# jaideepmurkute/Inference-Efficient-Vision-Models

Hardware: NVIDIA B200
Metric: pruned-INT8 ResNet-18 images/s @bs256 per GPU (synthetic 3x224x224) (higher is better)
Workload: dtype u8

## Files before the change

inference-efficient-vision-models_b200/csrc/conv_dual.cuh:

```cuda
#pragma once
#include "conv_tc.cuh"

namespace ievm {

struct ConvDualParams {
  void* out;
  const float* ep0;
  const float* ep1;
  int out_zp, out_lo;
  int fast_round;
  int relu;
  int32_t* dump_acc;
  float epc0[kEpConst];
  float epc1[kEpConst];
};

template <int kDtype, int kCluster>
__global__ void __launch_bounds__(kConvThreads, 1)
conv_dual_kernel(const __grid_constant__ CUtensorMap tmap_a, const __grid_constant__ CUtensorMap tmap_b,
                 const __grid_constant__ CUtensorMap tmap_b2, const __grid_constant__ ConvTcParams p,
                 const __grid_constant__ ConvDualParams x) {
  extern __shared__ uint8_t smem_raw[];
  const uint32_t raw_addr = smem_u32(smem_raw);
  uint8_t* smem = smem_raw + ((1024u - (raw_addr & 1023u)) & 1023u);

  const int kw = p.kw != 0 ? p.kw : p.ksize;
  const int stride_w = p.kw != 0 ? p.stride_w : p.stride;
  const int pad_w = p.kw != 0 ? p.pad_w : p.pad;
  const int num_kb = p.ksize * kw * p.kchunks;
  const int a_bytes = p.a_stage_bytes;
  const int b_bytes = (p.bn / kCluster) * p.kc_bytes;
  const int G = p.kb_group;
  const int slots = p.stages * G;
  const int b_slots = p.resident_b ? num_kb + p.kchunks : slots;
  uint8_t* sA = smem;
  uint8_t* sB = smem + slots * a_bytes;
  float* s_ep = reinterpret_cast<float*>(sB + b_slots * b_bytes);
  uint64_t* full_bar = reinterpret_cast<uint64_t*>(s_ep + 4 * p.cout_pad);
  uint64_t* empty_bar = full_bar + p.stages;
  uint64_t* tfull_bar = empty_bar + p.stages;
  uint64_t* tempty_bar = tfull_bar + kMaxAcc;
  uint64_t* bres_bar = tempty_bar + kMaxAcc;
  uint32_t* tmem_slot = reinterpret_cast<uint32_t*>(bres_bar + 1);

// ... 36 lines not shown
  tc_fence_before();
  __syncthreads();
  if (kCluster > 1) cluster_sync_all();
  tc_fence_after();
  const uint32_t tmem_base = *reinterpret_cast<volatile uint32_t*>(tmem_slot);
  griddep_launch_dependents();

  const int class_tiles = kCluster > 1 ? ((p.m_tiles + kCluster - 1) / kCluster) * p.n_tiles : p.m_tiles * p.n_tiles;
  const int total_tiles = 2 * class_tiles;
  const int tile_first = kCluster > 1 ? static_cast<int>(blockIdx.x) / kCluster : static_cast<int>(blockIdx.x);
  const int tile_step = kCluster > 1 ? static_cast<int>(gridDim.x) / kCluster : static_cast<int>(gridDim.x);
  const int hw = p.ho * p.wo;
  const int ctr_y = p.ksize >> 1, ctr_x = kw >> 1;

  if (warp == 0) {
    if (p.resident_b && elect_one()) {
      mbar_expect_tx(bres_bar, static_cast<uint32_t>((num_kb + p.kchunks) * b_bytes));
      for (int kb = 0; kb < num_kb; ++kb) tma_load_2d(sB + kb * b_bytes, &tmap_b, bres_bar, kb * p.kc_elems, 0);
      for (int ch = 0; ch < p.kchunks; ++ch)
        tma_load_2d(sB + (num_kb + ch) * b_bytes, &tmap_b2, bres_bar, ch * p.kc_elems, 0);
    }
    __syncwarp();
    griddep_wait_conv();
    const uint32_t tx_bytes = static_cast<uint32_t>(p.resident_b ? p.a_tx_bytes : p.a_tx_bytes + b_bytes);
    int stage = 0;
    uint32_t phase = 0;
    for (int tile = tile_first; tile < total_tiles; tile += tile_step) {
      const bool cls1 = tile >= class_tiles;
      const int ct = cls1 ? tile - class_tiles : tile;
      const int m_group = ct / p.n_tiles;
      const int n_tile = ct - m_group * p.n_tiles;
      const int m_tile = kCluster > 1 ? m_group * kCluster + static_cast<int>(crank) : m_group;
      const int m0 = m_tile * kTileM;
      const int img = fast_div(m0, hw, p.hw_magic);
      const int rem = m0 - img * hw;
      const int oy = fast_div(rem, p.wo, p.wo_magic);
      const int ox = rem - oy * p.wo;
      const int base_w = ox * stride_w - pad_w;
      const int base_h = oy * p.stride - p.pad;
      const int ty_lo = cls1 ? ctr_y : 0, ty_hi = cls1 ? ctr_y + 1 : p.ksize;
      const int tx_lo = cls1 ? ctr_x : 0, tx_hi = cls1 ? ctr_x + 1 : kw;
      const int nkb = cls1 ? p.kchunks : num_kb;
      const CUtensorMap* wmap = cls1 ? &tmap_b2 : &tmap_b;
      int kb = 0, g = 0;
      for (int ty = ty_lo; ty < ty_hi; ++ty) {
        for (int tx = tx_lo; tx < tx_hi; ++tx) {
// ... 41 lines not shown
    const uint32_t b_step = static_cast<uint32_t>(b_bytes) >> 4;
    const uint32_t idesc = p.idesc;
    auto mma = [&](uint32_t d, uint32_t a_lo, uint32_t b_lo, uint32_t accum) {
      if (kCluster > 1) {
        if (kDtype == kDtypeI8) umma_i8_lohi_pair(d, a_lo, b_lo, hi, idesc, accum);
        else umma_f16_lohi_pair(d, a_lo, b_lo, hi, idesc, accum);
      } else {
        if (kDtype == kDtypeI8) umma_i8_lohi(d, a_lo, b_lo, hi, idesc, accum);
        else umma_f16_lohi(d, a_lo, b_lo, hi, idesc, accum);
      }
    };
    if (p.resident_b) wait_or_die(bres_bar, 0, 0x500u, p.stuck_flag);
    for (int tile = tile_first; leader && tile < total_tiles; tile += tile_step) {
      const bool cls1 = tile >= class_tiles;
      const int nkb = cls1 ? p.kchunks : num_kb;
      const int b_first = cls1 ? num_kb : 0;
      wait_or_die(&tempty_bar[acc], acc_phase ^ 1u, 0x200u | acc, p.stuck_flag);
      tc_fence_after();
      const uint32_t d_tmem = tmem_base + static_cast<uint32_t>(acc * p.acc_stride);
      for (int kb0 = 0; kb0 < nkb; kb0 += G) {
        const int cnt = min(G, nkb - kb0);
        wait_or_die(&full_bar[stage], phase, 0x300u | stage, p.stuck_flag);
        tc_fence_after();
        if (elect_one()) {
          for (int g = 0; g < cnt; ++g) {
            const int kb = kb0 + g;
            const uint32_t a_lo = a_lo0 + static_cast<uint32_t>(stage * G + g) * a_step;
            const uint32_t b_lo = b_lo0 + static_cast<uint32_t>(p.resident_b ? b_first + kb : stage * G + g) * b_step;
            mma(d_tmem, a_lo, b_lo, kb != 0 ? 1u : 0u);
            mma(d_tmem, a_lo + 2, b_lo + 2, 1u);
            if (wide) {
              mma(d_tmem, a_lo + 4, b_lo + 4, 1u);
              mma(d_tmem, a_lo + 6, b_lo + 6, 1u);
            }
          }
          const bool last = kb0 + cnt == nkb;
          if (kCluster > 1) {
            umma_commit_pair(&empty_bar[stage]);
            if (last) umma_commit_pair(&tfull_bar[acc]);
          } else {
            umma_commit(&empty_bar[stage]);
            if (last) umma_commit(&tfull_bar[acc]);
          }
        }
        __syncwarp();
        if (++stage == p.stages) {
          stage = 0;
          phase ^= 1u;
        }
      }
      if (++acc == p.nacc) {
        acc = 0;
        acc_phase ^= 1u;
      }
    }
  } else {
    const int quad = warp & 3;
    const int groups = p.nacc < kGroupsMax ? p.nacc : kGroupsMax;
    const int group = ((warp - 2) >> 2) & (groups - 1);
    const int sub = ((warp - 2) >> 2) / groups;
    const int csub = kGroupsMax / groups;
    const int row = quad * 32 + lane;
    const int nchunks = p.bn >> 4;
    griddep_wait_conv();
    int acc_next = 0, seq = 0;
    uint32_t acc_phase_next = 0;
    for (int tile = tile_first; tile < total_tiles; tile += tile_step, ++seq) {
      const int acc = acc_next;
      const uint32_t acc_phase = acc_phase_next;
      if (++acc_next == p.nacc) {
        acc_next = 0;
        acc_phase_next ^= 1u;
      }
      if ((seq & (groups - 1)) != group) continue;
      const bool cls1 = tile >= class_tiles;
      const int ct = cls1 ? tile - class_tiles : tile;
      const int m_group = ct / p.n_tiles;
      const int n_tile = ct - m_group * p.n_tiles;
      const int m_tile = kCluster > 1 ? m_group * kCluster + static_cast<int>(crank) : m_group;
      const int m = m_tile * kTileM + row;
      const bool valid = m < p.m_total;
      const int n0 = n_tile * p.bn;
      uint8_t* out_row = static_cast<uint8_t*>(cls1 ? x.out : p.out) +
                         static_cast<size_t>(m) * p.out_pitch * (kDtype == kDtypeI8 ? 1 : 2);
      const float* e0 = s_ep + (cls1 ? 2 * p.cout_pad : 0);
      const float* e1 = e0 + p.cout_pad;
      const int zp = cls1 ? x.out_zp : p.out_zp;
      const int lo = cls1 ? x.out_lo : p.out_lo;
      const bool fast = (cls1 ? x.fast_round : p.fast_round) != 0;
      const bool relu = (cls1 ? x.relu : p.relu) != 0;
      int32_t* dump = cls1 ? x.dump_acc : p.dump_acc;

      wait_or_die(&tfull_bar[acc], acc_phase, 0x400u | acc, p.stuck_flag);
      tc_fence_after();
      const uint32_t t_row = tmem_base + (static_cast<uint32_t>(quad * 32) << 16) + static_cast<uint32_t>(acc * p.acc_stride);
      uint32_t va[16], vb[16];
      auto chunk = [&](const uint32_t (&v)[16], int c) {
        const int ch = n0 + c * 16;
        if (valid && dump != nullptr) {
          int4* d = reinterpret_cast<int4*>(dump + static_cast<size_t>(m) * p.dump_pitch + ch);
#pragma unroll
          for (int j = 0; j < 4; ++j)
            d[j] = make_int4(static_cast<int>(v[4 * j]), static_cast<int>(v[4 * j + 1]), static_cast<int>(v[4 * j + 2]),
                             static_cast<int>(v[4 * j + 3]));
        }
        if (kDtype == kDtypeI8) {
          const uint4 o = fast ? epilogue16_i8<true>(v, e0 + ch, e1 + ch, zp, lo) : epilogue16_i8<false>(v, e0 + ch, e1 + ch, zp, lo);
          if (valid) *reinterpret_cast<uint4*>(out_row + ch) = o;
        } else {
          __half* op = reinterpret_cast<__half*>(out_row) + ch;
          if (relu) epilogue16_f16<false, true>(v, e0 + ch, op, op, valid);
          else epilogue16_f16<false, false>(v, e0 + ch, op, op, valid);
        }
      };
      int c = sub;
      if (c < nchunks) tmem_ld_32x32b_x16(t_row + static_cast<uint32_t>(c * 16), va);
      while (c < nchunks) {
        tmem_ld_wait();
        if (c + csub < nchunks) tmem_ld_32x32b_x16(t_row + static_cast<uint32_t>((c + csub) * 16), vb);
        chunk(va, c);
        c += csub;
        if (c >= nchunks) break;
        tmem_ld_wait();
        if (c + csub < nchunks) tmem_ld_32x32b_x16(t_row + static_cast<uint32_t>((c + csub) * 16), va);
        chunk(vb, c);
        c += csub;
      }
      tc_fence_before();
      __syncwarp();
      if (lane == 0) {
        if (kCluster > 1 && !leader) mbar_arrive_remote(&tempty_bar[acc], 0u);
        else mbar_arrive(&tempty_bar[acc]);
      }
    }
  }

  tc_fence_before();
  __syncthreads();
  if (kCluster > 1) cluster_sync_all();
  if (warp == 1) {
    tc_fence_after();
    if (kCluster > 1) tmem_dealloc_pair(tmem_base, static_cast<uint32_t>(p.tmem_cols));
    else tmem_dealloc(tmem_base, static_cast<uint32_t>(p.tmem_cols));
  }
}

}
```

inference-efficient-vision-models_b200/csrc/conv_s2.cuh:

```cuda
#pragma once
#include "conv_dual.cuh"

namespace ievm {

__global__ void __launch_bounds__(kConvThreads, 1)
conv_s2_kernel(const __grid_constant__ CUtensorMap tmap_a, const __grid_constant__ CUtensorMap tmap_b,
               const __grid_constant__ CUtensorMap tmap_b2, const __grid_constant__ ConvTcParams p,
               const __grid_constant__ ConvDualParams x) {
  extern __shared__ uint8_t smem_raw[];
  const uint32_t raw_addr = smem_u32(smem_raw);
  uint8_t* smem = smem_raw + ((1024u - (raw_addr & 1023u)) & 1023u);

  constexpr int kRowBytes = 64;
  constexpr int kBlocks = 10;
  const int pb = p.phase_bytes;
  const int b_bytes = p.bn * kRowBytes;
  uint8_t* sA = smem;
  uint8_t* sB = smem + p.stages * p.a_stage_bytes + 1024;
  uint64_t* full_bar = reinterpret_cast<uint64_t*>(sB + kBlocks * b_bytes);
  uint64_t* empty_bar = full_bar + p.stages;
  uint64_t* tfull_bar = empty_bar + p.stages;
  uint64_t* tempty_bar = tfull_bar + kMaxAcc;
  uint64_t* bres_bar = tempty_bar + kMaxAcc;
  uint32_t* tmem_slot = reinterpret_cast<uint32_t*>(bres_bar + 1);

  const int warp = threadIdx.x >> 5;
  const int lane = threadIdx.x & 31;

  if (warp == 0 && lane == 0) {
    tma_prefetch_desc(&tmap_a);
    tma_prefetch_desc(&tmap_b);
// ... 15 lines not shown
  }
  tc_fence_before();
  __syncthreads();
  tc_fence_after();
  const uint32_t tmem_base = *reinterpret_cast<volatile uint32_t*>(tmem_slot);
  griddep_launch_dependents();

  int t_begin, t_end;
  {
    const int q = p.total_subs / static_cast<int>(gridDim.x), r = p.total_subs - q * static_cast<int>(gridDim.x);
    const int b = static_cast<int>(blockIdx.x);
    t_begin = b * q + (b < r ? b : r);
    t_end = t_begin + q + (b < r ? 1 : 0);
  }

  if (warp == 0) {
    if (elect_one()) {
      mbar_expect_tx(bres_bar, static_cast<uint32_t>(kBlocks * b_bytes));
      for (int kb = 0; kb < 9; ++kb) tma_load_2d(sB + kb * b_bytes, &tmap_b, bres_bar, kb * kRowBytes, 0);
      tma_load_2d(sB + 9 * b_bytes, &tmap_b2, bres_bar, 0, 0);
    }
    __syncwarp();
    griddep_wait_conv();
    int stage = 0;
    uint32_t phase = 0;
    int img = fast_div(t_begin, p.subs_per_img, p.spi_magic);
    int s = t_begin - img * p.subs_per_img;
    for (int t = t_begin; t < t_end; ++t) {
      wait_or_die(&empty_bar[stage], phase ^ 1u, 0x100u | stage, p.stuck_flag);
      if (elect_one()) {
        mbar_expect_tx(&full_bar[stage], static_cast<uint32_t>(p.a_tx_bytes));
        uint8_t* dst = sA + stage * p.a_stage_bytes;
        const int h0 = 2 * s * p.sub_rows - 2;
#pragma unroll
        for (int q = 0; q < 4; ++q) tma_load_4d(dst + q * pb, &tmap_a, &full_bar[stage], 0, (q & 1) - 2, h0 + (q >> 1), img);
      }
      __syncwarp();
      if (++stage == p.stages) {
        stage = 0;
        phase ^= 1u;
      }
      if (++s == p.subs_per_img) {
        s = 0;
        ++img;
      }
    }
  } else if (warp == 1) {
    int stage = 0;
    uint32_t phase = 0;
    const uint32_t hi = smem_desc_hi(kRowBytes);
    const uint32_t a_lo0 = smem_desc_lo(smem_u32(sA));
    const uint32_t b_lo0 = smem_desc_lo(smem_u32(sB));
    const uint32_t a_step = static_cast<uint32_t>(p.a_stage_bytes) >> 4;
    const uint32_t b_step = static_cast<uint32_t>(b_bytes) >> 4;
    const uint32_t pb16 = static_cast<uint32_t>(pb) >> 4;
    const uint32_t wp4 = static_cast<uint32_t>(p.wp) * (kRowBytes / 16);
    const uint32_t idesc = p.idesc;
    wait_or_die(bres_bar, 0, 0x500u, p.stuck_flag);
    for (int t = t_begin; t < t_end; ++t) {
      const int i = t - t_begin;
      const int acc0 = 2 * (i & 1);
      const uint32_t acc_par = (static_cast<uint32_t>(i >> 1) & 1u) ^ 1u;
      if (!mbar_try_wait5(&full_bar[stage], phase, &tempty_bar[acc0], acc_par, &tempty_bar[acc0 + 1], acc_par,
                          &tempty_bar[acc0 + 1], acc_par, &tempty_bar[acc0 + 1], acc_par)) {
        wait_or_die(&full_bar[stage], phase, 0x300u | stage, p.stuck_flag);
        wait_or_die(&tempty_bar[acc0], acc_par, 0x200u | acc0, p.stuck_flag);
        wait_or_die(&tempty_bar[acc0 + 1], acc_par, 0x200u | (acc0 + 1), p.stuck_flag);
      }
      tc_fence_after();
      if (elect_one()) {
        const uint32_t d0 = tmem_base + static_cast<uint32_t>(acc0 * p.acc_stride);
        const uint32_t d1 = d0 + static_cast<uint32_t>(p.acc_stride);
        const uint32_t a_base = a_lo0 + static_cast<uint32_t>(stage) * a_step;
#pragma unroll
        for (int tap = 0; tap < 9; ++tap) {
          const int ky = tap / 3, kx = tap % 3;
          const uint32_t ao = a_base + static_cast<uint32_t>((ky != 1 ? 2 : 0) + (kx != 1 ? 1 : 0)) * pb16 +
                              (ky != 0 ? wp4 : 0u) + (kx != 0 ? static_cast<uint32_t>(kRowBytes / 16) : 0u);
          const uint32_t bo = b_lo0 + static_cast<uint32_t>(tap) * b_step;
          umma_i8_lohi(d0, ao, bo, hi, idesc, tap != 0 ? 1u : 0u);
          umma_i8_lohi(d0, ao + 2, bo + 2, hi, idesc, 1u);
        }
        {
          const uint32_t ao = a_base + wp4 + static_cast<uint32_t>(kRowBytes / 16);
          const uint32_t bo = b_lo0 + 9u * b_step;
          umma_i8_lohi(d1, ao, bo, hi, idesc, 0u);
          umma_i8_lohi(d1, ao + 2, bo + 2, hi, idesc, 1u);
        }
        umma_commit(&tfull_bar[acc0]);
        umma_commit(&tfull_bar[acc0 + 1]);
        umma_commit(&empty_bar[stage]);
      }
      __syncwarp();
      if (++stage == p.stages) {
        stage = 0;
        phase ^= 1u;
      }
    }
  } else {
    const int quad = warp & 3;
    const int group = ((warp - 2) >> 2) & 3;
    const bool cls1 = (group & 1) != 0;
    const int row = quad * 32 + lane;
    const int r = fast_div(row, p.wp, p.wp_magic);
    const int c = row - r * p.wp;
    const bool pos_ok = row < p.sub_pos && c < p.wo;
    const int nchunks = p.bn >> 4;
    griddep_wait_conv();
    uint8_t* out_base = static_cast<uint8_t*>(cls1 ? x.out : p.out);
    const int zp = cls1 ? x.out_zp : p.out_zp;
    const int lo = cls1 ? x.out_lo : p.out_lo;
    const bool fast = (cls1 ? x.fast_round : p.fast_round) != 0;
    int32_t* dump = cls1 ? x.dump_acc : p.dump_acc;
    auto run = [&](auto fast_sel, const float* e0, const float* e1) __attribute__((always_inline)) {
      constexpr int kFs = decltype(fast_sel)::value;
      for (int i = group >> 1; t_begin + i < t_end; i += 2) {
        const int t = t_begin + i;
        const int acc = 2 * (i & 1) + (cls1 ? 1 : 0);
        const uint32_t acc_phase = static_cast<uint32_t>(i >> 1) & 1u;
        const int img = fast_div(t, p.subs_per_img, p.spi_magic);
        const int oy = (t - img * p.subs_per_img) * p.sub_rows + r;
        const bool valid = pos_ok && oy < p.ho;
        const int m = (img * p.ho + oy) * p.wo + c;
        uint8_t* out_row = out_base + static_cast<size_t>(m) * p.out_pitch;
        wait_or_die(&tfull_bar[acc], acc_phase, 0x400u | acc, p.stuck_flag);
        tc_fence_after();
        const uint32_t t_row = tmem_base + (static_cast<uint32_t>(quad * 32) << 16) + static_cast<uint32_t>(acc * p.acc_stride);
        uint32_t va[16], vb[16];
        auto chunk = [&](const uint32_t (&v)[16], int ch) {
          if (kFs < 0 && valid && dump != nullptr) {
            int4* d = reinterpret_cast<int4*>(dump + static_cast<size_t>(m) * p.dump_pitch + ch);
#pragma unroll
            for (int j = 0; j < 4; ++j)
              d[j] = make_int4(static_cast<int>(v[4 * j]), static_cast<int>(v[4 * j + 1]), static_cast<int>(v[4 * j + 2]),
                               static_cast<int>(v[4 * j + 3]));
          }
          uint4 o;
          if (kFs >= 0) o = epilogue16_i8<kFs == 1>(v, e0 + ch, e1 + ch, zp, lo);
          else o = fast ? epilogue16_i8<true>(v, e0 + ch, e1 + ch, zp, lo) : epilogue16_i8<false>(v, e0 + ch, e1 + ch, zp, lo);
          if (valid) *reinterpret_cast<uint4*>(out_row + ch) = o;
        };
        tmem_ld_32x32b_x16(t_row, va);
#pragma unroll 1
        for (int cc = 0; cc < nchunks; cc += 2) {
          tmem_ld_wait();
          if (cc + 1 < nchunks) tmem_ld_32x32b_x16(t_row + static_cast<uint32_t>((cc + 1) * 16), vb);
          chunk(va, cc * 16);
          if (cc + 1 >= nchunks) break;
          tmem_ld_wait();
          if (cc + 2 < nchunks) tmem_ld_32x32b_x16(t_row + static_cast<uint32_t>((cc + 2) * 16), va);
          chunk(vb, (cc + 1) * 16);
        }
        tc_fence_before();
        __syncwarp();
        if (lane == 0) mbar_arrive(&tempty_bar[acc]);
      }
    };
    auto dispatch = [&](const float* e0, const float* e1) {
      if (fast && dump == nullptr) run(std::integral_constant<int, 1>{}, e0, e1);
      else run(std::integral_constant<int, -1>{}, e0, e1);
    };
    if (cls1) dispatch(x.epc0, x.epc1);
    else dispatch(p.epc0, p.epc1);
  }

  tc_fence_before();
  __syncthreads();
  if (warp == 1) {
    tc_fence_after();
    tmem_dealloc(tmem_base, 512u);
  }
}

}
```

inference-efficient-vision-models_b200/csrc/conv_tc.cuh:

```cuda
#pragma once
#include <cuda_fp16.h>

#include <type_traits>

#include "ptx.cuh"

namespace ievm {

constexpr int kTileM = 128;
#ifndef IEVM_EPI_WARPS
#define IEVM_EPI_WARPS 16
#endif
constexpr int kEpiWarps = IEVM_EPI_WARPS;
constexpr int kEpiSub = kEpiWarps / 4;
constexpr int kEpiGroups = kEpiWarps / 4;
constexpr int kMaxAcc = 8;
constexpr int kConvThreads = 64 + 32 * kEpiWarps;

enum : int { kDtypeI8 = 0, kDtypeF16 = 1 };
enum : int { kModeIm2col = 0, kModeHalo = 1 };
constexpr int kMaxBandSubs = 4;
constexpr int kEpConst = 128;
constexpr int kHaloShapes = 4;
__host__ __device__ constexpr int halo_shape_wp(int s) { return s == 1 ? 58 : s == 2 ? 30 : s == 3 ? 58 : 0; }
// ... 75 lines not shown
      __trap();
    }
  }
}
__device__ __noinline__ void wait_or_die_slow(uint64_t* bar, uint32_t parity, uint32_t code, unsigned int* flag) {
  const uint64_t t0 = globaltimer_ns();
  uint32_t spins = 0;
  while (!mbar_try_wait(bar, parity)) {
    if ((++spins & 0x3ff) == 0 && globaltimer_ns() - t0 > IEVM_WAIT_LIMIT_NS) {
      if (flag) {
        *reinterpret_cast<volatile unsigned int*>(flag) = code;
        __threadfence_system();
      }
      __trap();
    }
  }
}
__device__ __forceinline__ void wait_or_die_ool(uint64_t* bar, uint32_t parity, uint32_t code, unsigned int* flag) {
  if (mbar_try_wait(bar, parity)) return;
  wait_or_die_slow(bar, parity, code, flag);
}

#ifdef IEVM_EXP_TIMING
constexpr int kExpSlots = 32, kExpCtas = 160, kExpWords = 16;
__device__ unsigned long long g_exp_timing[kExpSlots * kExpCtas * kExpWords];
#define IEVM_TIMED_WAIT(acc, ...)                 \
  do {                                            \
    const long long t__ = clock64();              \
    wait_or_die(__VA_ARGS__);                     \
    acc += clock64() - t__;                       \
  } while (0)
#else
#define IEVM_TIMED_WAIT(acc, ...) wait_or_die(__VA_ARGS__)
#endif

__device__ __forceinline__ int requant_i8(int acc, float bdiv, float mult, int zp, int lo) {
  const float v = __fmul_rn(__fadd_rn(__int2float_rn(acc), bdiv), mult);
  const int q = __float2int_rn(v) + zp;
  return min(max(q, lo), 255);
}
__device__ __forceinline__ int add_relu_i8(int aq, int a_zp, float a_scale, int rq, int r_zp, float r_scale,
                                           float inv_scale, int zp) {
  const float a = __fmaf_rn(a_scale, __int2float_rn(aq), __fmul_rn(a_scale, -__int2float_rn(a_zp)));
  const float b = __fmaf_rn(r_scale, __int2float_rn(rq), __fmul_rn(r_scale, -__int2float_rn(r_zp)));
  const float s = fmaxf(__fadd_rn(a, b), 0.0f);
  const int q = __float2int_rn(__fmul_rn(s, inv_scale)) + zp;
  return min(max(q, 0), 255);
}

__device__ __forceinline__ uint32_t pack_sat_u8(int a_hi, int b_lo, uint32_t c_upper) {
  uint32_t d;
  asm("cvt.pack.sat.u8.s32.b32 %0, %1, %2, %3;" : "=r"(d) : "r"(a_hi), "r"(b_lo), "r"(c_upper));
  return d;
}
__device__ __forceinline__ uint32_t pack4_sat_u8(int q0, int q1, int q2, int q3) {
  return pack_sat_u8(q1, q0, pack_sat_u8(q3, q2, 0u));
// ... 194 lines not shown
      o = p.fast_round ? epilogue16_i8_res<true, kResI2F>(v, r4, s_ep0 + ch, s_ep1 + ch, k)
                       : epilogue16_i8_res<false, kResI2F>(v, r4, s_ep0 + ch, s_ep1 + ch, k);
    } else {
      o = p.fast_round ? epilogue16_i8<true>(v, s_ep0 + ch, s_ep1 + ch, p.out_zp, p.out_lo)
                       : epilogue16_i8<false>(v, s_ep0 + ch, s_ep1 + ch, p.out_zp, p.out_lo);
    }
    if (valid) *reinterpret_cast<uint4*>(op) = o;
  } else {
    __half* op = static_cast<__half*>(p.out) + static_cast<size_t>(m) * p.out_pitch + ch;
    if (kHasRes) {
      if (p.relu) epilogue16_f16_pre<true>(v, s_ep0 + ch, r4, r4b, op, valid);
      else epilogue16_f16_pre<false>(v, s_ep0 + ch, r4, r4b, op, valid);
    } else {
      if (p.relu) epilogue16_f16<false, true>(v, s_ep0 + ch, op, op, valid);
      else epilogue16_f16<false, false>(v, s_ep0 + ch, op, op, valid);
    }
  }
}

template <int kDtype, bool kHasRes, int kMode, int kCluster, int kShape = 0, int kEpiW = kEpiWarps, bool kZc = false>
__global__ void __launch_bounds__(64 + 32 * kEpiW, kEpiW == 8 ? 2 : 1)
conv_tc_kernel(const __grid_constant__ CUtensorMap tmap_a, const __grid_constant__ CUtensorMap tmap_b,
               const __grid_constant__ ConvTcParams p) {
  extern __shared__ uint8_t smem_raw[];
  const uint32_t raw_addr = smem_u32(smem_raw);
  uint8_t* smem = smem_raw + ((1024u - (raw_addr & 1023u)) & 1023u);

  const int num_kb = p.ksize * p.ksize * p.kchunks;
  const int a_bytes = p.a_stage_bytes;
  const int b_bytes = (p.bn / kCluster) * p.kc_bytes;
  const int slots = p.stages * p.kb_group;
  const int b_slots = p.resident_b ? num_kb : slots;
  uint8_t* sA = smem;
  uint8_t* sB = smem + slots * a_bytes;
  float* s_ep0 = reinterpret_cast<float*>(sB + b_slots * b_bytes);
  float* s_ep1 = s_ep0 + p.cout_pad;
  uint64_t* full_bar = reinterpret_cast<uint64_t*>(s_ep1 + p.cout_pad);
  uint64_t* empty_bar = full_bar + p.stages;
  uint64_t* tfull_bar = empty_bar + p.stages;
  uint64_t* tempty_bar = tfull_bar + kMaxAcc;
  uint64_t* bres_bar = tempty_bar + kMaxAcc;
  uint32_t* tmem_slot = reinterpret_cast<uint32_t*>(bres_bar + 1);

  const int warp = threadIdx.x >> 5;
  const int lane = threadIdx.x & 31;

// ... 41 lines not shown
  const int hw = p.ho * p.wo;
  int t_begin = 0, t_end = 0;
  if (kMode == kModeHalo) {
    const int q = p.total_subs / static_cast<int>(gridDim.x), r = p.total_subs - q * static_cast<int>(gridDim.x);
    const int b = static_cast<int>(blockIdx.x);
    t_begin = b * q + (b < r ? b : r);
    t_end = t_begin + q + (b < r ? 1 : 0);
  }
#ifdef IEVM_EXP_TIMING
  long long tm_wait_a = 0, tm_wait_b = 0;
  const long long tm_t0 = clock64();
  const unsigned long long tm_ns0 = globaltimer_ns();
  unsigned long long* tm_out = g_exp_timing + (static_cast<size_t>(p.timing_slot) * kExpCtas + blockIdx.x) * kExpWords;
  int tm_tiles = 0;
#endif

  if (warp == 0) {
    if (p.resident_b && elect_one()) {
      mbar_expect_tx(bres_bar, static_cast<uint32_t>(num_kb * b_bytes));
      for (int kb = 0; kb < num_kb; ++kb) tma_load_2d(sB + kb * b_bytes, &tmap_b, bres_bar, kb * p.kc_elems, 0);
    }
    __syncwarp();
    griddep_wait_conv();
    const uint32_t tx_bytes = static_cast<uint32_t>(p.resident_b ? p.a_tx_bytes : p.a_tx_bytes + b_bytes);
    int stage = 0;
    uint32_t phase = 0;
    if (kMode == kModeHalo) {
      int img = fast_div(t_begin, p.subs_per_img, p.spi_magic);
      int s0 = t_begin - img * p.subs_per_img;
      for (int t = t_begin; t < t_end;) {
        const int ns = min(p.band_subs, min(p.subs_per_img - s0, t_end - t));
        IEVM_TIMED_WAIT(tm_wait_a, &empty_bar[stage], phase ^ 1u, 0x100u | stage, p.stuck_flag);
        if (elect_one()) {
          mbar_expect_tx(&full_bar[stage], tx_bytes);
          tma_load_4d(sA + stage * a_bytes, &tmap_a, &full_bar[stage], 0, -1, s0 * p.sub_rows - 1, img);
        }
        __syncwarp();
        if (++stage == p.stages) {
          stage = 0;
          phase ^= 1u;
        }
        t += ns;
        s0 += ns;
        if (s0 == p.subs_per_img) {
          s0 = 0;
          ++img;
// ... 114 lines not shown
              bars[j + 1] = bars[j];
              par[j + 1] = par[j];
            }
          }
#ifdef IEVM_EXP_TIMING
          const long long tw0 = clock64();
#endif
          if (!mbar_try_wait5(bars[0], par[0], bars[1], par[1], bars[2], par[2], bars[3], par[3], bars[4], par[4])) {
            const uint64_t t0 = globaltimer_ns();
            uint32_t spins = 0;
            while (!mbar_try_wait5(bars[0], par[0], bars[1], par[1], bars[2], par[2], bars[3], par[3], bars[4], par[4])) {
              if ((++spins & 0x3ff) == 0 && globaltimer_ns() - t0 > IEVM_WAIT_LIMIT_NS) {
                wait_or_die(bars[0], par[0], 0x300u | stage, p.stuck_flag);
#pragma unroll
                for (int j = 1; j <= kMaxBandSubs; ++j) wait_or_die(bars[j], par[j], 0x200u | j, p.stuck_flag);
              }
            }
          }
#ifdef IEVM_EXP_TIMING
          tm_wait_b += clock64() - tw0;
#endif
        }
        tc_fence_after();
        const uint32_t a_band = a_lo0 + static_cast<uint32_t>(stage) * a_step;
        if (elect_one()) {
          int a2 = acc;
#ifdef IEVM_EXP_TIMING
          const long long ti0 = clock64();
#endif
#pragma unroll 1
          for (int j = 0; j < ns; ++j) {
            const uint32_t d_tmem = tmem_base + static_cast<uint32_t>(a2 * p.acc_stride);
            const uint32_t a_lo = a_band + static_cast<uint32_t>(j) * sub_step;
            uint32_t b_base = b_lo0;
            asm volatile("" : "+r"(b_base));
#pragma unroll
            for (int tap = 0; tap < 9; ++tap) {
              const uint32_t ao = a_lo + static_cast<uint32_t>(tap / 3) * wp16 + static_cast<uint32_t>(tap % 3) * row16v;
              const uint32_t bo = b_base + static_cast<uint32_t>(tap) * bstep;
              mma(d_tmem, ao, bo, tap != 0 ? 1u : 0u);
              mma(d_tmem, ao + 2, bo + 2, 1u);
              if (widev) {
                mma(d_tmem, ao + 4, bo + 4, 1u);
                mma(d_tmem, ao + 6, bo + 6, 1u);
              }
            }
// ... 9 lines not shown
        {
          const int adv = acc + ns;
          acc_phase ^= (adv >= p.nacc) ? 1u : 0u;
          acc = adv >= p.nacc ? adv - p.nacc : adv;
        }
        if (++stage == p.stages) {
          stage = 0;
          phase ^= 1u;
        }
        t += ns;
        s0 += ns;
        if (s0 == p.subs_per_img) s0 = 0;
      }
    } else {
      const int G = p.kb_group;
      const int groups_per_tile = num_kb / G;
      for (int tile = tile_first; leader && tile < total_tiles; tile += tile_step) {
        IEVM_TIMED_WAIT(tm_wait_a, &tempty_bar[acc], acc_phase ^ 1u, 0x200u | acc, p.stuck_flag);
        tc_fence_after();
        const uint32_t d_tmem = tmem_base + static_cast<uint32_t>(acc * p.acc_stride);
        for (int kg = 0; kg < groups_per_tile; ++kg) {
          IEVM_TIMED_WAIT(tm_wait_b, &full_bar[stage], phase, 0x300u | stage, p.stuck_flag);
          tc_fence_after();
          if (elect_one()) {
            for (int g = 0; g < G; ++g) {
              const int kb = kg * G + g;
              const uint32_t a_lo = a_lo0 + static_cast<uint32_t>(stage * G + g) * a_step;
              const uint32_t b_lo = b_lo0 + static_cast<uint32_t>(p.resident_b ? kb : stage * G + g) * b_step;
              mma_kblock(d_tmem, a_lo, b_lo, kb != 0 ? 1u : 0u);
            }
            if (kCluster > 1) {
              umma_commit_pair(&empty_bar[stage]);
              if (kg == groups_per_tile - 1) umma_commit_pair(&tfull_bar[acc]);
            } else {
              umma_commit(&empty_bar[stage]);
              if (kg == groups_per_tile - 1) umma_commit(&tfull_bar[acc]);
            }
          }
          __syncwarp();
          if (++stage == p.stages) {
            stage = 0;
            phase ^= 1u;
          }
        }
        if (++acc == p.nacc) {
          acc = 0;
          acc_phase ^= 1u;
        }
      }
    }
#ifdef IEVM_EXP_TIMING
    for (int o = 16; o > 0; o >>= 1) {
      const long long other = __shfl_xor_sync(0xffffffffu, tm_wait_a, o);
      tm_wait_a = other > tm_wait_a ? other : tm_wait_a;
    }
    if (lane == 0 && blockIdx.x < kExpCtas) {
      tm_out[0] = clock64() - tm_t0;
      tm_out[1] = tm_wait_a;
      tm_out[2] = tm_wait_b;
      tm_out[3] = globaltimer_ns() - tm_ns0;
    }
#endif
  } else {
    const int quad = warp & 3;
    const int groups = p.nacc < kGroupsMax ? p.nacc : kGroupsMax;
    const int group = ((warp - 2) >> 2) & (groups - 1);
    const int sub = ((warp - 2) >> 2) / groups;
    const int csub = kGroupsMax / groups;
    const int row = quad * 32 + lane;
    const int nchunks = p.bn >> 4;
    griddep_wait_conv();
    AddReluConst k;
    k.lo_f = static_cast<float>(p.out_lo - p.out_zp);
    k.hi_f = static_cast<float>(255 - p.out_zp);
    k.a_scale = p.a_scale;
    k.r_scale = p.res_scale;
    k.inv_scale = p.inv_add_scale;
    k.pa = __fmul_rn(p.a_scale, -static_cast<float>(p.out_zp));
    k.pb = __fmul_rn(p.res_scale, -static_cast<float>(p.res_zp));
    k.lo_q = static_cast<float>(p.out_lo);
    k.zp_f = static_cast<float>(p.out_zp);
    k.add_zp = p.add_zp;
    k.c1_add = -kRoundMagicBits - (p.out_lo - p.out_zp);
    k.c1_max = 255 - p.out_lo;
    k.c2_add = -kRoundMagicBits;
    k.c2_max = 255 - p.add_zp;
    k.zp4 = static_cast<uint32_t>(p.add_zp) * 0x01010101u;
    const int sub_row = kMode == kModeHalo ? fast_div(row, p.wp, p.wp_magic) : 0;
    const int sub_x = row - sub_row * p.wp;
    const bool sub_ok = kMode == kModeHalo && row < p.sub_pos && sub_x < p.w_in;
    constexpr bool kResI8 = kHasRes && kDtype == kDtypeI8;
    constexpr bool kResF16 = kHasRes && kDtype == kDtypeF16;
    auto zcorr_row = [&](int oy, int ox) -> const int32_t* {
      int my = 0, mx = 0;
      for (int t = 0; t < p.ksize; ++t) {
        const int iy = oy * p.stride - p.pad + t, ix = ox * p.stride - p.pad + t;
        my |= (iy >= 0 && iy < p.h_in) ? (1 << t) : 0;
        mx |= (ix >= 0 && ix < p.w_in) ? (1 << t) : 0;
      }
      return p.zcorr + static_cast<size_t>((my << p.ksize) | mx) * p.cout_pad;
    };
    auto drain = [&](int acc, uint32_t acc_phase, int m, bool valid, int n0, const int32_t* zc = nullptr) {
      uint4 ra = make_uint4(0u, 0u, 0u, 0u), rb = ra;
      uint4 sa = ra, sb = ra;
      int c = sub;
      if (kResI8 && c < nchunks) ra = load_res16_i8(p, m, valid, n0 + c * 16);
      if (kResF16 && c < nchunks) load_res16_f16(p, m, valid, n0 + c * 16, ra, sa);
      IEVM_TIMED_WAIT(tm_wait_a, &tfull_bar[acc], acc_phase, 0x400u | acc, p.stuck_flag);
      tc_fence_after();
      const uint32_t t_row = tmem_base + (static_cast<uint32_t>(quad * 32) << 16) +
                             static_cast<uint32_t>(acc * p.acc_stride);
      uint32_t va[16], vb[16];
      if (c < nchunks) tmem_ld_32x32b_x16(t_row + static_cast<uint32_t>(c * 16), va);
      while (c < nchunks) {
        tmem_ld_wait();
        if (kZc && zc != nullptr) {
#pragma unroll
          for (int j = 0; j < 16; ++j) va[j] -= static_cast<uint32_t>(__ldg(zc + n0 + c * 16 + j));
        }
        if (c + csub < nchunks) {
          tmem_ld_32x32b_x16(t_row + static_cast<uint32_t>((c + csub) * 16), vb);
          if (kResI8) rb = load_res16_i8(p, m, valid, n0 + (c + csub) * 16);
          if (kResF16) load_res16_f16(p, m, valid, n0 + (c + csub) * 16, rb, sb);
        }
        epilogue_chunk<kDtype, kHasRes>(p, va, ra, m, valid, n0 + c * 16, s_ep0, s_ep1, k, sa);
        c += csub;
        if (c >= nchunks) break;
        tmem_ld_wait();
        if (kZc && zc != nullptr) {
#pragma unroll
          for (int j = 0; j < 16; ++j) vb[j] -= static_cast<uint32_t>(__ldg(zc + n0 + c * 16 + j));
        }
        if (c + csub < nchunks) {
          tmem_ld_32x32b_x16(t_row + static_cast<uint32_t>((c + csub) * 16), va);
          if (kResI8) ra = load_res16_i8(p, m, valid, n0 + (c + csub) * 16);
          if (kResF16) load_res16_f16(p, m, valid, n0 + (c + csub) * 16, ra, sa);
        }
        epilogue_chunk<kDtype, kHasRes>(p, vb, rb, m, valid, n0 + c * 16, s_ep0, s_ep1, k, sb);
        c += csub;
      }
      tc_fence_before();
      __syncwarp();
      if (lane == 0) {
        if (kCluster > 1 && !leader) mbar_arrive_remote(&tempty_bar[acc], 0u);
        else mbar_arrive(&tempty_bar[acc]);
      }
    };
    auto drain_static = [&](auto fast_sel, int acc, uint32_t acc_phase, int m, bool valid) {
      constexpr int kFs = kDtype == kDtypeI8 ? decltype(fast_sel)::value : -1;
      constexpr int kNch = kShape != 0 ? halo_shape_bn(kShape) / 16 : 1;
      uint4 rr[2];
      rr[0] = rr[1] = make_uint4(0u, 0u, 0u, 0u);
      uint4 rq[2];
      rq[0] = rq[1] = rr[0];
      if (kResI8) rr[0] = load_res16_i8(p, m, valid, 0);
      if (kResF16) load_res16_f16(p, m, valid, 0, rr[0], rq[0]);
      IEVM_TIMED_WAIT(tm_wait_a, &tfull_bar[acc], acc_phase, 0x400u | acc, p.stuck_flag);
      tc_fence_after();
      const uint32_t t_row = tmem_base + (static_cast<uint32_t>(quad * 32) << 16) +
                             static_cast<uint32_t>(acc * p.acc_stride);
      uint32_t vv[2][16];
      tmem_ld_32x32b_x16(t_row, vv[0]);
      if (kNch <= 4) {
#pragma unroll
        for (int c = 0; c < kNch; ++c) {
          tmem_ld_wait();
          if (c + 1 < kNch) {
            tmem_ld_32x32b_x16(t_row + static_cast<uint32_t>((c + 1) * 16), vv[(c + 1) & 1]);
            if (kResI8) rr[(c + 1) & 1] = load_res16_i8(p, m, valid, (c + 1) * 16);
            if (kResF16) load_res16_f16(p, m, valid, (c + 1) * 16, rr[(c + 1) & 1], rq[(c + 1) & 1]);
          }
          epilogue_chunk<kDtype, kHasRes, false, kFs>(p, vv[c & 1], rr[c & 1], m, valid, c * 16, p.epc0, p.epc1, k, rq[c & 1]);
        }
      } else {
#pragma unroll 1
        for (int c = 0; c < kNch; c += 2) {
          tmem_ld_wait();
          tmem_ld_32x32b_x16(t_row + static_cast<uint32_t>((c + 1) * 16), vv[1]);
          if (kResI8) rr[1] = load_res16_i8(p, m, valid, (c + 1) * 16);
          if (kResF16) load_res16_f16(p, m, valid, (c + 1) * 16, rr[1], rq[1]);
// ... 7 lines not shown
          epilogue_chunk<kDtype, kHasRes, true, kFs>(p, vv[1], rr[1], m, valid, (c + 1) * 16, p.epc0, p.epc1, k, rq[1]);
        }
      }
      tc_fence_before();
      __syncwarp();
      if (lane == 0) mbar_arrive(&tempty_bar[acc]);
    };
    if (kMode == kModeHalo) {
      const int nacc_shift = 31 - __clz(p.nacc);
      for (int t = t_begin + group; t < t_end; t += groups) {
        const int seq = t - t_begin;
        const int acc = seq & (p.nacc - 1);
        const uint32_t acc_phase = static_cast<uint32_t>(seq >> nacc_shift) & 1u;
#ifdef IEVM_EXP_TIMING
        ++tm_tiles;
#endif
        const int img = fast_div(t, p.subs_per_img, p.spi_magic);
        const int oy = (t - img * p.subs_per_img) * p.sub_rows + sub_row;
        const bool valid = sub_ok && oy < p.h_in;
        const int m = (img * p.h_in + oy) * p.w_in + sub_x;
        if (kShape != 0) {
          if (p.fast_round) drain_static(std::integral_constant<int, 1>{}, acc, acc_phase, m, valid);
          else drain_static(std::integral_constant<int, 0>{}, acc, acc_phase, m, valid);
        } else drain(acc, acc_phase, m, valid, 0, kZc ? zcorr_row(oy, sub_x) : nullptr);
      }
    } else {
      int acc_next = 0, seq = 0;
      uint32_t acc_phase_next = 0;
      for (int tile = tile_first; tile < total_tiles; tile += tile_step, ++seq) {
        const int acc = acc_next;
        const uint32_t acc_phase = acc_phase_next;
        if (++acc_next == p.nacc) {
          acc_next = 0;
          acc_phase_next ^= 1u;
        }
        if ((seq & (groups - 1)) != group) continue;
#ifdef IEVM_EXP_TIMING
        ++tm_tiles;
#endif
        const int m_group = tile / p.n_tiles;
        const int n_tile = tile - m_group * p.n_tiles;
        const int m_tile = kCluster > 1 ? m_group * kCluster + static_cast<int>(crank) : m_group;
        const int m = m_tile * kTileM + row;
        const int32_t* zc = nullptr;
        if (kZc) {
          const int rem = m - (m / hw) * hw;
          zc = zcorr_row(rem / p.wo, rem - (rem / p.wo) * p.wo);
        }
        drain(acc, acc_phase, m, m < p.m_total, n_tile * p.bn, zc);
      }
    }
  }

#ifdef IEVM_EXP_TIMING
  if (warp == 2 && lane == 0 && blockIdx.x < kExpCtas) {
    tm_out[6] = clock64() - tm_t0;
    tm_out[7] = tm_wait_a;
    tm_out[8] = tm_tiles;
  }
#endif
  tc_fence_before();
  __syncthreads();
#ifdef IEVM_EXP_TIMING
  if (warp == 1 && lane == 0 && blockIdx.x < kExpCtas) {
    tm_out[9] = clock64() - tm_t0;
    tm_out[10] = globaltimer_ns() - tm_ns0;
  }
#endif
  if (kCluster > 1) cluster_sync_all();
  if (warp == 1) {
    tc_fence_after();
    if (kCluster > 1) tmem_dealloc_pair(tmem_base, static_cast<uint32_t>(p.tmem_cols));
    else tmem_dealloc(tmem_base, static_cast<uint32_t>(p.tmem_cols));
  }
}

}
```

Baseline: 464,800.

## Split the final tiles' epilogue drain across all epilogue warp groups

In the dual, stride-2 and generic tensor-core conv kernels, the last few tiles of each CTA are now drained from TMEM by every epilogue warp group. Each group takes an interleaved subset of column chunks, instead of one group handling each tile alone. Only the owning group arrives on the accumulator-empty barrier. The goal is to shorten the per-CTA tail, where most epilogue warps sit idle while one group finishes the last accumulator. Phase-timing probes are also added, but they compile to nothing unless experimental timing is enabled.

```diff
diff --git a/inference-efficient-vision-models_b200/csrc/conv_dual.cuh b/inference-efficient-vision-models_b200/csrc/conv_dual.cuh
--- a/inference-efficient-vision-models_b200/csrc/conv_dual.cuh
+++ b/inference-efficient-vision-models_b200/csrc/conv_dual.cuh
@@ -20,6 +20,7 @@
 conv_dual_kernel(const __grid_constant__ CUtensorMap tmap_a, const __grid_constant__ CUtensorMap tmap_b,
                  const __grid_constant__ CUtensorMap tmap_b2, const __grid_constant__ ConvTcParams p,
                  const __grid_constant__ ConvDualParams x) {
+  IEVM_EXP_PHASE(const unsigned long long tm_start = globaltimer_ns();)
   extern __shared__ uint8_t smem_raw[];
   const uint32_t raw_addr = smem_u32(smem_raw);
   uint8_t* smem = smem_raw + ((1024u - (raw_addr & 1023u)) & 1023u);
@@ -102,6 +103,7 @@
     }
     __syncwarp();
     griddep_wait_conv();
+    IEVM_EXP_PHASE(exp_phase_stamp(p.timing_slot, 1);)
     const uint32_t tx_bytes = static_cast<uint32_t>(p.resident_b ? p.a_tx_bytes : p.a_tx_bytes + b_bytes);
     int stage = 0;
     uint32_t phase = 0;
@@ -189,6 +191,7 @@
         const int cnt = min(G, nkb - kb0);
         wait_or_die(&full_bar[stage], phase, 0x300u | stage, p.stuck_flag);
         tc_fence_after();
+        IEVM_EXP_PHASE(if (tile == tile_first && kb0 == 0) exp_phase_stamp(p.timing_slot, 2);)
         if (elect_one()) {
           for (int g = 0; g < cnt; ++g) {
             const int kb = kb0 + g;
@@ -224,12 +227,16 @@
   } else {
     const int quad = warp & 3;
     const int groups = p.nacc < kGroupsMax ? p.nacc : kGroupsMax;
-    const int group = ((warp - 2) >> 2) & (groups - 1);
-    const int sub = ((warp - 2) >> 2) / groups;
+    const int qsub = (warp - 2) >> 2;
+    const int group = qsub & (groups - 1);
+    const int sub = qsub / groups;
     const int csub = kGroupsMax / groups;
     const int row = quad * 32 + lane;
     const int nchunks = p.bn >> 4;
     griddep_wait_conv();
+    IEVM_EXP_PHASE(unsigned long long tm_commit = 0;)
+    const int ntiles = tile_first < total_tiles ? (total_tiles - tile_first + tile_step - 1) / tile_step : 0;
+    const int fin0 = ntiles - groups;
     int acc_next = 0, seq = 0;
     uint32_t acc_phase_next = 0;
     for (int tile = tile_first; tile < total_tiles; tile += tile_step, ++seq) {
@@ -239,7 +246,10 @@
         acc_next = 0;
         acc_phase_next ^= 1u;
       }
-      if ((seq & (groups - 1)) != group) continue;
+      const bool own = (seq & (groups - 1)) == group;
+      const bool fin = seq >= fin0;
+      if (!own && !fin) continue;
+      const int c0 = fin ? qsub : sub, cstep = fin ? kGroupsMax : csub;
       const bool cls1 = tile >= class_tiles;
       const int ct = cls1 ? tile - class_tiles : tile;
       const int m_group = ct / p.n_tiles;
@@ -259,6 +269,7 @@
       int32_t* dump = cls1 ? x.dump_acc : p.dump_acc;
 
       wait_or_die(&tfull_bar[acc], acc_phase, 0x400u | acc, p.stuck_flag);
+      IEVM_EXP_PHASE(tm_commit = globaltimer_ns();)
       tc_fence_after();
       const uint32_t t_row = tmem_base + (static_cast<uint32_t>(quad * 32) << 16) + static_cast<uint32_t>(acc * p.acc_stride);
       uint32_t va[16], vb[16];
@@ -280,26 +291,27 @@
           else epilogue16_f16<false, false>(v, e0 + ch, op, op, valid);
         }
       };
-      int c = sub;
+      int c = c0;
       if (c < nchunks) tmem_ld_32x32b_x16(t_row + static_cast<uint32_t>(c * 16), va);
       while (c < nchunks) {
         tmem_ld_wait();
-        if (c + csub < nchunks) tmem_ld_32x32b_x16(t_row + static_cast<uint32_t>((c + csub) * 16), vb);
+        if (c + cstep < nchunks) tmem_ld_32x32b_x16(t_row + static_cast<uint32_t>((c + cstep) * 16), vb);
         chunk(va, c);
-        c += csub;
+        c += cstep;
         if (c >= nchunks) break;
         tmem_ld_wait();
-        if (c + csub < nchunks) tmem_ld_32x32b_x16(t_row + static_cast<uint32_t>((c + csub) * 16), va);
+        if (c + cstep < nchunks) tmem_ld_32x32b_x16(t_row + static_cast<uint32_t>((c + cstep) * 16), va);
         chunk(vb, c);
-        c += csub;
+        c += cstep;
       }
       tc_fence_before();
       __syncwarp();
-      if (lane == 0) {
+      if (own && lane == 0) {
         if (kCluster > 1 && !leader) mbar_arrive_remote(&tempty_bar[acc], 0u);
         else mbar_arrive(&tempty_bar[acc]);
       }
     }
+    IEVM_EXP_PHASE(exp_phase_epilogue_done(p.timing_slot, tm_commit);)
   }
 
   tc_fence_before();
@@ -309,6 +321,7 @@
     tc_fence_after();
     if (kCluster > 1) tmem_dealloc_pair(tmem_base, static_cast<uint32_t>(p.tmem_cols));
     else tmem_dealloc(tmem_base, static_cast<uint32_t>(p.tmem_cols));
+    IEVM_EXP_PHASE(exp_phase_exit(p.timing_slot, tm_start);)
   }
 }
 
diff --git a/inference-efficient-vision-models_b200/csrc/conv_s2.cuh b/inference-efficient-vision-models_b200/csrc/conv_s2.cuh
--- a/inference-efficient-vision-models_b200/csrc/conv_s2.cuh
+++ b/inference-efficient-vision-models_b200/csrc/conv_s2.cuh
@@ -7,6 +7,7 @@
 conv_s2_kernel(const __grid_constant__ CUtensorMap tmap_a, const __grid_constant__ CUtensorMap tmap_b,
                const __grid_constant__ CUtensorMap tmap_b2, const __grid_constant__ ConvTcParams p,
                const __grid_constant__ ConvDualParams x) {
+  IEVM_EXP_PHASE(const unsigned long long tm_start = globaltimer_ns();)
   extern __shared__ uint8_t smem_raw[];
   const uint32_t raw_addr = smem_u32(smem_raw);
   uint8_t* smem = smem_raw + ((1024u - (raw_addr & 1023u)) & 1023u);
@@ -68,6 +69,7 @@
     }
     __syncwarp();
     griddep_wait_conv();
+    IEVM_EXP_PHASE(exp_phase_stamp(p.timing_slot, 1);)
     int stage = 0;
     uint32_t phase = 0;
     int img = fast_div(t_begin, p.subs_per_img, p.spi_magic);
@@ -114,6 +116,7 @@
         wait_or_die(&tempty_bar[acc0 + 1], acc_par, 0x200u | (acc0 + 1), p.stuck_flag);
       }
       tc_fence_after();
+      IEVM_EXP_PHASE(if (i == 0) exp_phase_stamp(p.timing_slot, 2);)
       if (elect_one()) {
         const uint32_t d0 = tmem_base + static_cast<uint32_t>(acc0 * p.acc_stride);
         const uint32_t d1 = d0 + static_cast<uint32_t>(p.acc_stride);
@@ -158,9 +161,14 @@
     const int lo = cls1 ? x.out_lo : p.out_lo;
     const bool fast = (cls1 ? x.fast_round : p.fast_round) != 0;
     int32_t* dump = cls1 ? x.dump_acc : p.dump_acc;
+    IEVM_EXP_PHASE(unsigned long long tm_commit = 0;)
     auto run = [&](auto fast_sel, const float* e0, const float* e1) __attribute__((always_inline)) {
       constexpr int kFs = decltype(fast_sel)::value;
-      for (int i = group >> 1; t_begin + i < t_end; i += 2) {
+      const int n = t_end - t_begin;
+      for (int i = n > 0 ? min(group >> 1, n - 1) : 0; i < n;) {
+        const bool fin = i == n - 1;
+        const bool own = (i & 1) == (group >> 1);
+        const int c0 = fin ? group >> 1 : 0, cstep = fin ? 2 : 1;
         const int t = t_begin + i;
         const int acc = 2 * (i & 1) + (cls1 ? 1 : 0);
         const uint32_t acc_phase = static_cast<uint32_t>(i >> 1) & 1u;
@@ -170,6 +178,7 @@
         const int m = (img * p.ho + oy) * p.wo + c;
         uint8_t* out_row = out_base + static_cast<size_t>(m) * p.out_pitch;
         wait_or_die(&tfull_bar[acc], acc_phase, 0x400u | acc, p.stuck_flag);
+        IEVM_EXP_PHASE(tm_commit = globaltimer_ns();)
         tc_fence_after();
         const uint32_t t_row = tmem_base + (static_cast<uint32_t>(quad * 32) << 16) + static_cast<uint32_t>(acc * p.acc_stride);
         uint32_t va[16], vb[16];
@@ -186,20 +195,21 @@
           else o = fast ? epilogue16_i8<true>(v, e0 + ch, e1 + ch, zp, lo) : epilogue16_i8<false>(v, e0 + ch, e1 + ch, zp, lo);
           if (valid) *reinterpret_cast<uint4*>(out_row + ch) = o;
         };
-        tmem_ld_32x32b_x16(t_row, va);
+        tmem_ld_32x32b_x16(t_row + static_cast<uint32_t>(c0 * 16), va);
 #pragma unroll 1
-        for (int cc = 0; cc < nchunks; cc += 2) {
+        for (int cc = c0; cc < nchunks; cc += 2 * cstep) {
           tmem_ld_wait();
-          if (cc + 1 < nchunks) tmem_ld_32x32b_x16(t_row + static_cast<uint32_t>((cc + 1) * 16), vb);
+          if (cc + cstep < nchunks) tmem_ld_32x32b_x16(t_row + static_cast<uint32_t>((cc + cstep) * 16), vb);
           chunk(va, cc * 16);
-          if (cc + 1 >= nchunks) break;
+          if (cc + cstep >= nchunks) break;
           tmem_ld_wait();
-          if (cc + 2 < nchunks) tmem_ld_32x32b_x16(t_row + static_cast<uint32_t>((cc + 2) * 16), va);
-          chunk(vb, (cc + 1) * 16);
+          if (cc + 2 * cstep < nchunks) tmem_ld_32x32b_x16(t_row + static_cast<uint32_t>((cc + 2 * cstep) * 16), va);
+          chunk(vb, (cc + cstep) * 16);
         }
         tc_fence_before();
         __syncwarp();
-        if (lane == 0) mbar_arrive(&tempty_bar[acc]);
+        if (own && lane == 0) mbar_arrive(&tempty_bar[acc]);
+        i = fin ? n : (i + 2 < n - 1 ? i + 2 : n - 1);
       }
     };
     auto dispatch = [&](const float* e0, const float* e1) {
@@ -208,6 +218,7 @@
     };
     if (cls1) dispatch(x.epc0, x.epc1);
     else dispatch(p.epc0, p.epc1);
+    IEVM_EXP_PHASE(exp_phase_epilogue_done(p.timing_slot, tm_commit);)
   }
 
   tc_fence_before();
@@ -215,6 +226,7 @@
   if (warp == 1) {
     tc_fence_after();
     tmem_dealloc(tmem_base, 512u);
+    IEVM_EXP_PHASE(exp_phase_exit(p.timing_slot, tm_start);)
   }
 }
 
diff --git a/inference-efficient-vision-models_b200/csrc/conv_tc.cuh b/inference-efficient-vision-models_b200/csrc/conv_tc.cuh
--- a/inference-efficient-vision-models_b200/csrc/conv_tc.cuh
+++ b/inference-efficient-vision-models_b200/csrc/conv_tc.cuh
@@ -121,8 +121,29 @@
 }
 
 #ifdef IEVM_EXP_TIMING
-constexpr int kExpSlots = 32, kExpCtas = 160, kExpWords = 16;
+constexpr int kExpSlots = 32, kExpCtas = 296, kExpWords = 24, kExpPhase = 16;
 __device__ unsigned long long g_exp_timing[kExpSlots * kExpCtas * kExpWords];
+__device__ __forceinline__ unsigned long long* exp_timing_cta(int slot) {
+  return g_exp_timing + (static_cast<size_t>(slot) * kExpCtas + blockIdx.x) * kExpWords;
+}
+__device__ __forceinline__ void exp_phase_epilogue_done(int slot, unsigned long long t_commit) {
+  if ((threadIdx.x & 31) == 0 && blockIdx.x < kExpCtas) {
+    unsigned long long* o = exp_timing_cta(slot);
+    atomicMax(o + kExpPhase + 3, t_commit);
+    atomicMax(o + kExpPhase + 4, static_cast<unsigned long long>(globaltimer_ns()));
+  }
+}
+__device__ __forceinline__ void exp_phase_stamp(int slot, int word) {
+  if ((threadIdx.x & 31) == 0 && blockIdx.x < kExpCtas) exp_timing_cta(slot)[kExpPhase + word] = globaltimer_ns();
+}
+__device__ __forceinline__ void exp_phase_exit(int slot, unsigned long long t_start) {
+  if ((threadIdx.x & 31) == 0 && blockIdx.x < kExpCtas) {
+    unsigned long long* o = exp_timing_cta(slot);
+    o[kExpPhase] = t_start;
+    o[kExpPhase + 5] = globaltimer_ns();
+  }
+}
+#define IEVM_EXP_PHASE(...) __VA_ARGS__
 #define IEVM_TIMED_WAIT(acc, ...)                 \
   do {                                            \
     const long long t__ = clock64();              \
@@ -131,6 +152,7 @@
   } while (0)
 #else
 #define IEVM_TIMED_WAIT(acc, ...) wait_or_die(__VA_ARGS__)
+#define IEVM_EXP_PHASE(...)
 #endif
 
 __device__ __forceinline__ int requant_i8(int acc, float bdiv, float mult, int zp, int lo) {
@@ -371,6 +393,7 @@
 __global__ void __launch_bounds__(64 + 32 * kEpiW, kEpiW == 8 ? 2 : 1)
 conv_tc_kernel(const __grid_constant__ CUtensorMap tmap_a, const __grid_constant__ CUtensorMap tmap_b,
                const __grid_constant__ ConvTcParams p) {
+  IEVM_EXP_PHASE(const unsigned long long tm_start = globaltimer_ns();)
   extern __shared__ uint8_t smem_raw[];
   const uint32_t raw_addr = smem_u32(smem_raw);
   uint8_t* smem = smem_raw + ((1024u - (raw_addr & 1023u)) & 1023u);
@@ -458,6 +481,7 @@
     }
     __syncwarp();
     griddep_wait_conv();
+    IEVM_EXP_PHASE(exp_phase_stamp(p.timing_slot, 1);)
     const uint32_t tx_bytes = static_cast<uint32_t>(p.resident_b ? p.a_tx_bytes : p.a_tx_bytes + b_bytes);
     int stage = 0;
     uint32_t phase = 0;
@@ -618,6 +642,7 @@
 #endif
         }
         tc_fence_after();
+        IEVM_EXP_PHASE(if (t == t_begin) exp_phase_stamp(p.timing_slot, 2);)
         const uint32_t a_band = a_lo0 + static_cast<uint32_t>(stage) * a_step;
         if (elect_one()) {
           int a2 = acc;
@@ -673,6 +698,7 @@
         for (int kg = 0; kg < groups_per_tile; ++kg) {
           IEVM_TIMED_WAIT(tm_wait_b, &full_bar[stage], phase, 0x300u | stage, p.stuck_flag);
           tc_fence_after();
+          IEVM_EXP_PHASE(if (tile == tile_first && kg == 0) exp_phase_stamp(p.timing_slot, 2);)
           if (elect_one()) {
             for (int g = 0; g < G; ++g) {
               const int kb = kg * G + g;
@@ -715,8 +741,9 @@
   } else {
     const int quad = warp & 3;
     const int groups = p.nacc < kGroupsMax ? p.nacc : kGroupsMax;
-    const int group = ((warp - 2) >> 2) & (groups - 1);
-    const int sub = ((warp - 2) >> 2) / groups;
+    const int qsub = (warp - 2) >> 2;
+    const int group = qsub & (groups - 1);
+    const int sub = qsub / groups;
     const int csub = kGroupsMax / groups;
     const int row = quad * 32 + lane;
     const int nchunks = p.bn >> 4;
@@ -742,6 +769,7 @@
     const bool sub_ok = kMode == kModeHalo && row < p.sub_pos && sub_x < p.w_in;
     constexpr bool kResI8 = kHasRes && kDtype == kDtypeI8;
     constexpr bool kResF16 = kHasRes && kDtype == kDtypeF16;
+    IEVM_EXP_PHASE(unsigned long long tm_commit = 0;)
     auto zcorr_row = [&](int oy, int ox) -> const int32_t* {
       int my = 0, mx = 0;
       for (int t = 0; t < p.ksize; ++t) {
@@ -751,13 +779,15 @@
       }
       return p.zcorr + static_cast<size_t>((my << p.ksize) | mx) * p.cout_pad;
     };
-    auto drain = [&](int acc, uint32_t acc_phase, int m, bool valid, int n0, const int32_t* zc = nullptr) {
+    auto drain = [&](int acc, uint32_t acc_phase, int m, bool valid, int n0, const int32_t* zc, int c0, int cstep,
+                     bool arrive) {
       uint4 ra = make_uint4(0u, 0u, 0u, 0u), rb = ra;
       uint4 sa = ra, sb = ra;
-      int c = sub;
+      int c = c0;
       if (kResI8 && c < nchunks) ra = load_res16_i8(p, m, valid, n0 + c * 16);
       if (kResF16 && c < nchunks) load_res16_f16(p, m, valid, n0 + c * 16, ra, sa);
       IEVM_TIMED_WAIT(tm_wait_a, &tfull_bar[acc], acc_phase, 0x400u | acc, p.stuck_flag);
+      IEVM_EXP_PHASE(tm_commit = globaltimer_ns();)
       tc_fence_after();
       const uint32_t t_row = tmem_base + (static_cast<uint32_t>(quad * 32) << 16) +
                              static_cast<uint32_t>(acc * p.acc_stride);
@@ -769,30 +799,30 @@
 #pragma unroll
           for (int j = 0; j < 16; ++j) va[j] -= static_cast<uint32_t>(__ldg(zc + n0 + c * 16 + j));
         }
-        if (c + csub < nchunks) {
-          tmem_ld_32x32b_x16(t_row + static_cast<uint32_t>((c + csub) * 16), vb);
-          if (kResI8) rb = load_res16_i8(p, m, valid, n0 + (c + csub) * 16);
-          if (kResF16) load_res16_f16(p, m, valid, n0 + (c + csub) * 16, rb, sb);
+        if (c + cstep < nchunks) {
+          tmem_ld_32x32b_x16(t_row + static_cast<uint32_t>((c + cstep) * 16), vb);
+          if (kResI8) rb = load_res16_i8(p, m, valid, n0 + (c + cstep) * 16);
+          if (kResF16) load_res16_f16(p, m, valid, n0 + (c + cstep) * 16, rb, sb);
         }
         epilogue_chunk<kDtype, kHasRes>(p, va, ra, m, valid, n0 + c * 16, s_ep0, s_ep1, k, sa);
-        c += csub;
+        c += cstep;
         if (c >= nchunks) break;
         tmem_ld_wait();
         if (kZc && zc != nullptr) {
 #pragma unroll
           for (int j = 0; j < 16; ++j) vb[j] -= static_cast<uint32_t>(__ldg(zc + n0 + c * 16 + j));
         }
-        if (c + csub < nchunks) {
-          tmem_ld_32x32b_x16(t_row + static_cast<uint32_t>((c + csub) * 16), va);
-          if (kResI8) ra = load_res16_i8(p, m, valid, n0 + (c + csub) * 16);
-          if (kResF16) load_res16_f16(p, m, valid, n0 + (c + csub) * 16, ra, sa);
+        if (c + cstep < nchunks) {
+          tmem_ld_32x32b_x16(t_row + static_cast<uint32_t>((c + cstep) * 16), va);
+          if (kResI8) ra = load_res16_i8(p, m, valid, n0 + (c + cstep) * 16);
+          if (kResF16) load_res16_f16(p, m, valid, n0 + (c + cstep) * 16, ra, sa);
         }
         epilogue_chunk<kDtype, kHasRes>(p, vb, rb, m, valid, n0 + c * 16, s_ep0, s_ep1, k, sb);
-        c += csub;
+        c += cstep;
       }
       tc_fence_before();
       __syncwarp();
-      if (lane == 0) {
+      if (arrive && lane == 0) {
         if (kCluster > 1 && !leader) mbar_arrive_remote(&tempty_bar[acc], 0u);
         else mbar_arrive(&tempty_bar[acc]);
       }
@@ -807,6 +837,7 @@
       if (kResI8) rr[0] = load_res16_i8(p, m, valid, 0);
       if (kResF16) load_res16_f16(p, m, valid, 0, rr[0], rq[0]);
       IEVM_TIMED_WAIT(tm_wait_a, &tfull_bar[acc], acc_phase, 0x400u | acc, p.stuck_flag);
+      IEVM_EXP_PHASE(tm_commit = globaltimer_ns();)
       tc_fence_after();
       const uint32_t t_row = tmem_base + (static_cast<uint32_t>(quad * 32) << 16) +
                              static_cast<uint32_t>(acc * p.acc_stride);
@@ -860,9 +891,11 @@
         if (kShape != 0) {
           if (p.fast_round) drain_static(std::integral_constant<int, 1>{}, acc, acc_phase, m, valid);
           else drain_static(std::integral_constant<int, 0>{}, acc, acc_phase, m, valid);
-        } else drain(acc, acc_phase, m, valid, 0, kZc ? zcorr_row(oy, sub_x) : nullptr);
+        } else drain(acc, acc_phase, m, valid, 0, kZc ? zcorr_row(oy, sub_x) : nullptr, sub, csub, true);
       }
     } else {
+      const int ntiles = tile_first < total_tiles ? (total_tiles - tile_first + tile_step - 1) / tile_step : 0;
+      const int fin0 = ntiles - groups;
       int acc_next = 0, seq = 0;
       uint32_t acc_phase_next = 0;
       for (int tile = tile_first; tile < total_tiles; tile += tile_step, ++seq) {
@@ -872,7 +905,9 @@
           acc_next = 0;
           acc_phase_next ^= 1u;
         }
-        if ((seq & (groups - 1)) != group) continue;
+        const bool own = (seq & (groups - 1)) == group;
+        const bool fin = seq >= fin0;
+        if (!own && !fin) continue;
 #ifdef IEVM_EXP_TIMING
         ++tm_tiles;
 #endif
@@ -885,9 +920,10 @@
           const int rem = m - (m / hw) * hw;
           zc = zcorr_row(rem / p.wo, rem - (rem / p.wo) * p.wo);
         }
-        drain(acc, acc_phase, m, m < p.m_total, n_tile * p.bn, zc);
-      }
-    }
+        drain(acc, acc_phase, m, m < p.m_total, n_tile * p.bn, zc, fin ? qsub : sub, fin ? kGroupsMax : csub, own);
+      }
+    }
+    IEVM_EXP_PHASE(exp_phase_epilogue_done(p.timing_slot, tm_commit);)
   }
 
 #ifdef IEVM_EXP_TIMING
@@ -910,7 +946,8 @@
     tc_fence_after();
     if (kCluster > 1) tmem_dealloc_pair(tmem_base, static_cast<uint32_t>(p.tmem_cols));
     else tmem_dealloc(tmem_base, static_cast<uint32_t>(p.tmem_cols));
-  }
-}
-
-}
+    IEVM_EXP_PHASE(exp_phase_exit(p.timing_slot, tm_start);)
+  }
+}
+
+}
```

Result: no change. 464,600, median of 6 (-0.0%).
